# yhhshb/biolib

Hardware: AMD Instinct MI355X
Metric: Gbp/s minimizer-scanned (k=31,w=11) (higher is better)
Workload: dtype u64

## Files before the change

biolib_amd/csrc/bl_capi.hip:

```cpp
#include <hip/hip_runtime.h>
#include <algorithm>
#include <cstdio>
#include <cstdlib>
#include <cstring>
#include <deque>
#include <new>
#include <string>
#include <utility>
#include <vector>

#include "../../include/biolib_amd.h"
#include "bl_host.hpp"
#include "bl_launch.hpp"
#include "bl_lookup_launch.hpp"
#include "bl_read_counts_launch.hpp"
#include "bl_scan128_launch.hpp"

namespace {

thread_local std::string g_err;

int fail(int code, const std::string& msg)
{
    g_err = msg;
// ... 34 lines not shown
    size_t ws_bytes = 0;
    unsigned char* tile_buf = nullptr;
    size_t tile_buf_bytes = 0;
    uint16_t* slot_buf = nullptr;
    size_t slot_buf_bytes = 0;
    hipEvent_t ev_start = nullptr, ev_stop = nullptr;
    hipEvent_t ev_count_done = nullptr;
    bool count_recorded = false;
    bool scan_recorded = false;

    unsigned long long* shards() const { return reinterpret_cast<unsigned long long*>(ws + HDR_BYTES); }
    unsigned long long* result() const { return reinterpret_cast<unsigned long long*>(ws + HDR_BYTES + SHARD_BYTES); }
};

struct bl_ctx {
    int device = 0;
    Lane lanes[2];
    Lane* cur = nullptr;
    int next_lane = 0;
    int n_lanes = 1;
    uint32_t emit_lds_per_wg = 0;
    hipStream_t user_stream = nullptr;
    bool borrowed = false;
    hipStream_t stream = nullptr;
    unsigned long long* pinned = nullptr;
    hipEvent_t slot_ev[RING] = {};
    int next_slot = 0;
    std::deque<Pending> pending;
    bool timed = false;
    bool exact_windows = false;
    bool position_tiled = false;
    bool packed_codes = true;
    bool direct_codes = true;
    int jaccard128_path = 0;
    bool count128_tables = true;
    int table_prefix_bits = -1;
    bool ktiming = false;
    bl::LaunchLog last_kernels{};
    std::vector<hipEvent_t> ev_pool;
    std::vector<std::pair<hipEvent_t, hipEvent_t>> ev_open;
    double kernel_ms = 0.0;
    uint64_t kernel_launches = 0;
    std::vector<std::pair<hipEvent_t, hipEvent_t>> marks;
    std::vector<bl_batch*> batches;
    void* scratch[8] = {};
    size_t scratch_bytes[8] = {};
    std::vector<std::pair<void*, size_t>> pool_idle;
    std::vector<std::pair<void*, size_t>> pool_live;

    unsigned long long* shards() const { return cur->shards(); }
    unsigned long long* result() const { return cur->result(); }
    static size_t fixed_bytes() { return HDR_BYTES + SHARD_BYTES + RESULT_WORDS * sizeof(unsigned long long); }
};

struct bl_batch {
    bl_ctx* ctx = nullptr;
    uint8_t* bases = nullptr;
    bool owns_bases = false;
    uint32_t* start_bits = nullptr;
    uint32_t* packed = nullptr;
    uint32_t* codes = nullptr;
    uint32_t* chunk_bad = nullptr;
    uint64_t n_bases = 0;
    uint64_t n_seqs = 0;
    uint64_t read_len = 0;
    uint64_t origin = 0;
// ... 437 lines not shown

int bl_ctx_last_scan_ms(bl_ctx* c, float* ms)
{
    if (!c || !ms) return fail(BL_ERR_INVALID, "NULL argument");
    if (!c->timed) return fail(BL_ERR_INVALID, "no scan has been issued on this context");
    BL_HIP(hipEventSynchronize(c->cur->ev_stop));
    BL_HIP(hipEventElapsedTime(ms, c->cur->ev_start, c->cur->ev_stop));
    return BL_OK;
}

int bl_ctx_set_exact_windows(bl_ctx* c, int on)
{
    if (!c) return fail(BL_ERR_INVALID, "ctx is NULL");
    c->exact_windows = on != 0;
    return BL_OK;
}

int bl_ctx_set_option(bl_ctx* c, const char* name, int64_t value)
{
    if (!c || !name) return fail(BL_ERR_INVALID, "bl_ctx_set_option: NULL argument");
    const std::string n(name);
    if (n == "exact_windows" && (value == 0 || value == 1)) return bl_ctx_set_exact_windows(c, (int)value);
    if (n == "lanes") return bl_ctx_set_lanes(c, (int)value);
    if (n == "position_tiled" && (value == 0 || value == 1)) {
        c->position_tiled = value != 0;
        return BL_OK;
    }
    if (n == "packed_codes" && (value == 0 || value == 1)) {
        c->packed_codes = value != 0;
        return BL_OK;
    }
    if (n == "direct_codes" && (value == 0 || value == 1)) {
        c->direct_codes = value != 0;
        return BL_OK;
    }
    if (n == "count128_tables" && (value == 0 || value == 1)) {
        c->count128_tables = value != 0;
        return BL_OK;
    }
    if (n == "jaccard128_path" && value >= 0 && value <= 2) {
        c->jaccard128_path = (int)value;
        return BL_OK;
    }
    if (n == "table_prefix_bits" && value >= -1 && value <= bllk::MAX_PREFIX_BITS) {
        c->table_prefix_bits = (int)value;
        return BL_OK;
    }
    if (n == "emit_lds_bytes" && value >= 0 && value <= 160 * 1024) {
        c->emit_lds_per_wg = (uint32_t)value;
        return BL_OK;
    }
    return fail(BL_ERR_INVALID, "bl_ctx_set_option: unknown name or value out of range: " + n);
}

int bl_ctx_kernel_timing(bl_ctx* c, int enable)
{
    if (!c) return fail(BL_ERR_INVALID, "ctx is NULL");
    int rc = sync_ctx(c);
    if (rc != BL_OK) return rc;
    c->ktiming = enable != 0;
    c->kernel_ms = 0.0;
    c->kernel_launches = 0;
    return BL_OK;
}

int bl_ctx_kernel_time(bl_ctx* c, double* total_ms, uint64_t* launches)
// ... 527 lines not shown
{
    if (!c || !b || b->ctx != c) return fail(BL_ERR_INVALID, "ctx/batch is NULL or the batch belongs to another context");
    c->last_kernels.n = 0;
    if (unit < 1 || unit > bl::MAX_UNIT) return fail(BL_ERR_INVALID, "hashed unit length must be in [1, 32]");
    if (w < 1 || w > bl::MAX_W) return fail(BL_ERR_INVALID, "window must be in [1, 64]");
    uint64_t end;
    int rc = blh::range_end(b->n_bases, first, n, "a scan range", end);
    if (rc != BL_OK) return rc;
    if (end <= first) return zero_result(c, result, flags);
    p.bases = b->bases;
    p.n_bases = (int64_t)b->n_bases;
    p.pos_base = (int64_t)b->origin;
    p.exact_windows = c->exact_windows ? 1 : 0;
    bl::plan_scan(mode, (int64_t)first, (int64_t)end, (int)w, p);
    if (b->read_len && !c->position_tiled && !p.use_threshold && bl::frl_width_built(mode, (int)w)) {
        bl::plan_scan_frl_for(mode, (int64_t)first, (int64_t)end, (int64_t)b->n_bases, (int64_t)b->read_len, (int)unit, (int)w, (flags & BL_FLAG_CANONICAL) != 0, p);
    }
    if (!p.frl) {
        rc = ensure_start_bits(c, b);
        if (rc != BL_OK) return rc;
    }
    p.start_bits = b->start_bits;
    if (c->packed_codes && b->codes && bl::packed_covers(p) && (p.frl || bl::packed_scan_shape(mode, (int)w))) {
        p.codes_packed = b->codes;
        p.chunk_bad = b->chunk_bad;
        p.direct_codes = c->direct_codes ? 1 : 0;
    }
    p.unit = (int32_t)unit;
    p.w = (int32_t)w;
    p.seed = (uint32_t)seed;
    p.canonical = (flags & BL_FLAG_CANONICAL) ? 1 : 0;
    p.drop_last = (flags & BL_FLAG_DROP_LAST) ? 1 : 0;
    p.capacity = capacity;
    rc = begin_scan(c);
    if (rc != BL_OK) return rc;
    const size_t nt = (size_t)p.n_tiles, nb = (nt + bl::SCAN_BLK - 1) / bl::SCAN_BLK;
    rc = grow(c, reinterpret_cast<void**>(&c->cur->tile_buf), &c->cur->tile_buf_bytes, (2 * nt + 2 * nb + 8) * sizeof(unsigned long long) + nt * sizeof(uint32_t));
    if (rc != BL_OK) return rc;
    const size_t n_lists = mode == bl::MODE_SUPERKMER ? 3 : 1;
    const size_t slot_entries = nt * (size_t)p.stride;
    const size_t list_bytes = n_lists * slot_entries * sizeof(uint16_t);
    const size_t code_bytes = p.codes_packed ? 0 : nt * (size_t)p.slot_chunks * sizeof(uint32_t);
    rc = grow(c, reinterpret_cast<void**>(&c->cur->slot_buf), &c->cur->slot_buf_bytes, list_bytes + code_bytes);
    if (rc != BL_OK) return rc;
    unsigned long long* tb = reinterpret_cast<unsigned long long*>(c->cur->tile_buf);
    p.tile_counts = tb;
    p.tile_base = tb + nt;
    unsigned long long* block_tot = tb + 2 * nt;
    p.block_base = block_tot + nb;
    p.redo_list = reinterpret_cast<uint32_t*>(tb + 2 * nt + 2 * nb + 8);
    p.redo_count = reinterpret_cast<unsigned long long*>(c->cur->ws) + 1;
    p.slots_a = c->cur->slot_buf;
    p.slots_j = mode == bl::MODE_SUPERKMER ? c->cur->slot_buf + slot_entries : nullptr;
    p.slots_e = mode == bl::MODE_SUPERKMER ? c->cur->slot_buf + 2 * slot_entries : nullptr;
    p.slots_c = p.codes_packed ? nullptr : reinterpret_cast<uint32_t*>(reinterpret_cast<unsigned char*>(c->cur->slot_buf) + list_bytes);
    p.shards = c->shards();
    const bl::GroupRange all{0, (uint32_t)p.n_tiles};
    unsigned long long* carry = reinterpret_cast<unsigned long long*>(c->cur->ws);
    const bool staggered = c->n_lanes == 2 && !c->borrowed;
    if (staggered) {
        Lane* other = c->cur == &c->lanes[0] ? &c->lanes[1] : &c->lanes[0];
        if (other->count_recorded) BL_HIP(hipStreamWaitEvent(c->stream, other->ev_count_done, 0));
    }
    rc = kernel_event(c, true);
    if (rc != BL_OK) return rc;
    hipError_t e = bl::launch_scan_count(mode, p, all, c->stream, &c->last_kernels);
    if (e != hipSuccess) return fail(BL_ERR_HIP, std::string("scan_count_kernel: ") + hipGetErrorString(e));
    if (staggered) {
        BL_HIP(hipEventRecord(c->cur->ev_count_done, c->stream));
        c->cur->count_recorded = true;
    }
    rc = kernel_event(c, false);
    if (rc != BL_OK) return rc;
    e = bl::launch_tile_scan(p, all, block_tot, carry, c->stream);
    if (e != hipSuccess) return fail(BL_ERR_HIP, std::string("tile_scan: ") + hipGetErrorString(e));
    const uint32_t emit_lds_default = mode == bl::MODE_SUPERKMER ? 8192u : 28672u;
    e = bl::launch_scan_emit(mode, p, all, c->stream, staggered ? (c->emit_lds_per_wg ? c->emit_lds_per_wg : emit_lds_default) : 0, &c->last_kernels);
    if (e != hipSuccess) return fail(BL_ERR_HIP, std::string("scan_emit_kernel: ") + hipGetErrorString(e));
    return BL_OK;
}

int bl_scan_minimizers(bl_ctx* c, const bl_batch* b, uint64_t first, uint64_t n, uint32_t unit, uint32_t w, uint64_t seed, uint32_t flags,
                       uint64_t* d_values, uint64_t* d_positions, uint64_t* d_hashes, uint64_t capacity, bl_result* result)
{
    bl::ScanParams p{};
    p.out_value = d_values;
    p.out_pos = d_positions;
    p.out_hash = d_hashes;
    const bool wants = d_values || d_positions || d_hashes;
    int rc = scan_windows(bl::MODE_MINIMIZER, c, b, first, n, unit, w, seed, flags, p, wants ? capacity : 0, result);
    if (rc != BL_OK || p.n_tiles == 0) return rc;
    return end_scan(c, 1u << 0, result, wants, capacity, flags);
}

int bl_scan_hash_sample(bl_ctx* c, const bl_batch* b, uint64_t first, uint64_t n, uint32_t k, uint64_t seed, uint64_t threshold, uint32_t flags,
                        uint64_t* d_values, uint64_t* d_positions, uint64_t* d_hashes, uint64_t capacity, bl_result* result)
{
    bl::ScanParams p{};
    p.out_value = d_values;
    p.out_pos = d_positions;
    p.out_hash = d_hashes;
    p.use_threshold = 1;
// ... 164 lines not shown
```

biolib_amd/csrc/bl_kernels.hip:

```cpp
#include <hip/hip_runtime.h>
#include <cstdlib>
#include "bl_scan_frl.hpp"
#include "bl_launch.hpp"

#ifndef BL_SY0_WAVES
#define BL_SY0_WAVES 2
#endif
#ifndef BL_SY2_WAVES
#define BL_SY2_WAVES 3
#endif
#ifndef BL_CS_WAVES
#define BL_CS_WAVES 3
#endif
#ifndef BL_POSAX_WAVES
#define BL_POSAX_WAVES 4
#endif
#ifndef BL_SKAX_WAVES
#define BL_SKAX_WAVES 4
#endif
#ifndef BL_C4_WAVES
#define BL_C4_WAVES 5
#endif
#ifndef BL_CSRT_WAVES
#define BL_CSRT_WAVES 3
#endif

namespace bl {


__device__ __forceinline__ uint32_t wave_incl_scan_u32(uint32_t v, int lane)
{
    (void)lane;
#ifndef BL_SCAN_BUILTIN_DPP
// ... 170 lines not shown
        if (!PACKED) {
            uint32_t* sc = p.slots_c + (size_t)tile * p.slot_chunks;
            for (int c = tid; c < p.slot_chunks; c += TPB) sc[c] = sh.codes[c];
        }
        __syncthreads();
    }

    ThreadState st;
    bool tie = false;
    phase_hash_frl<MODE, W, NS, GENERIC, APPROX, U>(p, sh, tid, q0, tile, st, clean ? p.codes_packed + (q0 >> 4) : nullptr);
    phase_window_frl_a<MODE, W, NS, LIM_LAST, APPROX>(p, sh, tid, st, nullptr, &tie, clean);
    if (APPROX) {
        const bool any = wave_any(tie);
        if ((tid & 63) == 0) sh.wave_redo[wave_index(tid)] = any ? 1u : 0u;
    }
    const uint32_t packed = phase_window_frl_b<MODE, W, NS>(p, tid, st, nullptr);

    uint32_t total;
    const uint32_t excl = block_excl_scan(packed, sh.wave_tot, tid, total);
    const uint32_t n_s = total & 0xffffu, n_e = total >> 16;
    phase_list_frl<MODE, W, NS>(sh, st, excl & 0xffffu, excl >> 16);
    if (tid == 0) p.tile_counts[tile] = (unsigned long long)n_s | ((unsigned long long)n_e << 32);
    __syncthreads();
    if (APPROX && tid == 0 && BL_COLD((sh.wave_redo[0] | sh.wave_redo[1] | sh.wave_redo[2] | sh.wave_redo[3]) != 0)) p.redo_list[atomicAdd(p.redo_count, 1ull)] = tile;
    const size_t slot = (size_t)tile * p.stride;
    spill_list(p.slots_a + slot, sh.list_a, n_s, tid);
    if (MODE == MODE_SUPERKMER) {
        spill_list(p.slots_j + slot, sh.list_j, n_s, tid);
        spill_list(p.slots_e + slot, sh.list_e, n_e, tid);
    }
}

constexpr int C3_RC = NCHUNK + 4;
template <int MODE, bool LOOPED = false, bool C3 = false, bool WIDE = false, bool PACKED = false>
__device__ __forceinline__ void emit_tile(const ScanParams& p, uint32_t* codes, uint32_t tile, int tid, Digest& dg)
{
    const int64_t q0 = tile_q0(p, tile);
    const size_t slot = (size_t)tile * p.stride;
    const unsigned long long cnt = uniform64(p.tile_counts[tile]);
    const unsigned long long base = uniform64(p.tile_base[tile] + p.block_base[tile / SCAN_BLK]);
    const int needed = staged_chunks(p);
    const uint32_t* sc = PACKED ? p.codes_packed + (q0 >> 4) : p.slots_c + (size_t)tile * p.slot_chunks;
    const uint32_t c0 = (MODE != MODE_SYNCMER && tid < needed) ? sc[tid] : 0;
    const uint32_t c1 = (MODE != MODE_SYNCMER && TPB + tid < needed) ? sc[TPB + tid] : 0;
    const uint16_t* la = p.slots_a + slot;
    const uint16_t* lj = MODE == MODE_SUPERKMER ? p.slots_j + slot : nullptr;
    const bool in0 = tid < p.stride, in1 = TPB + tid < p.stride;
    const uint32_t a0 = in0 ? la[tid] : 0, a1 = in1 ? la[TPB + tid] : 0;
    uint32_t j0 = 0, j1 = 0;
    if (MODE == MODE_SUPERKMER) {
        j0 = in0 ? lj[tid] : 0;
        j1 = in1 ? lj[TPB + tid] : 0;
    }
    const uint32_t n_s = (uint32_t)cnt, n_e = (uint32_t)(cnt >> 32);
    if (n_s == 0 && n_e == 0) {
        if (LOOPED && MODE != MODE_SYNCMER) __syncthreads();
        return;
    }
    const uint64_t base_s = base & 0xffffffffull, base_e = base >> 32;
    if (C3) {
        if (tid < needed) {
            codes[1 + tid] = c0;
            codes[C3_RC + needed - tid] = revcomp16(c0);
        }
        if (TPB + tid < needed) {
            codes[1 + TPB + tid] = c1;
            codes[C3_RC + needed - TPB - tid] = revcomp16(c1);
        }
        __syncthreads();
    } else if (MODE != MODE_SYNCMER) {
        if (tid < needed) codes[tid] = c0;
        if (TPB + tid < needed) codes[TPB + tid] = c1;
        __syncthreads();
    }
    const bool fits = !BL_COLD(base_s + n_s > p.capacity);
    TileLists L{codes, la, lj, MODE == MODE_SUPERKMER ? p.slots_e + slot : nullptr, MODE == MODE_SUPERKMER ? p.slots_e + slot + p.stride : nullptr};
    const uint32_t d = (uint32_t)(base_s - base_e);
    auto one = [&](uint32_t r, uint32_t ent, uint32_t ent_j) {
        const Record rec = C3 ? emit_prepare_c3<LOOPED>(p, codes + 1, codes + C3_RC + 1, needed, q0, ent, dg) : emit_prepare<MODE, LOOPED>(p, codes, q0, ent, ent_j, dg);
        if (fits) emit_store<MODE, false>(p, rec, base_s + r);
        else emit_store<MODE, true>(p, rec, base_s + r);
        if (MODE == MODE_SUPERKMER && (p.out_size || p.out_records) && (fits || base_s + r < p.capacity)) {
            const int size = (int)(end_position(p, L, tile, q0, r + d, n_e) - (int64_t)rec.first + 1);
            if (p.out_size) p.out_size[base_s + r] = (uint8_t)size;
            if (WIDE) {
                if (p.out_records) emit_record128(p, codes, needed - 1, q0, rec, size, base_s + r);
            } else if (p.out_records) {
                emit_record(p, codes, needed - 1, q0, rec, size, base_s + r);
            }
        }
    };
    if ((uint32_t)tid < n_s) one(tid, a0, j0);
    if (LOOPED) BL_SCHED_FENCE();
    if ((uint32_t)(TPB + tid) < n_s) one(TPB + tid, a1, j1);
    if (LOOPED) BL_SCHED_FENCE();
#pragma unroll 1
    for (uint32_t r = 2 * TPB + tid; r < n_s; r += TPB) one(r, la[r], MODE == MODE_SUPERKMER ? lj[r] : 0u);
}

template <bool PACKED, int MODE, int W, int U, int C, int SY = 0>
__global__ __launch_bounds__(TPB, (MODE == MODE_MINIMIZER && SY == 2 ? BL_POSAX_WAVES : MODE == MODE_SUPERKMER && SY == 2 ? BL_SKAX_WAVES : SY == 1 && W < 0 ? BL_CSRT_WAVES : SY == 1 ? BL_CS_WAVES : SY == 2 ? BL_SY2_WAVES : (MODE == MODE_SYNCMER && W > 0 ? BL_SY0_WAVES : MODE == MODE_SYNCMER || (MODE == MODE_SUPERKMER && W == -32) ? 2 : (W == -32 || (W < 0 && MODE == MODE_SUPERKMER) ? 3 : (W == -16 ? 5 : (W < 0 ? 4 : (W <= 11 ? 5 : (MODE == MODE_SUPERKMER && W == 17 && U == 15 ? BL_C4_WAVES : 4)))))))) void scan_count_kernel(const ScanParams pin, GroupRange g)
{
    __shared__ TileShared<MODE, W> sh;
    ScanParams p = pin;
    if (U != 0) p.unit = U;
    if (W > 0) {
        p.w = W;
        p.stride = NWAVE * (64 * S - 16 * ((W + 15) / 16));
    }
// ... 45 lines not shown
#ifndef BL_FRL_WAVES
#define BL_FRL_WAVES 5
#endif
template <bool PACKED, int MODE, int W, int NS, int U, int L, int C, bool APPROX = false>
__global__ __launch_bounds__(TPB, (W <= 11 ? BL_FRL_WAVES : 4)) void scan_count_frl_kernel(const ScanParams pin, GroupRange g)
{
    __shared__ TileShared<MODE, W> sh;
    const ScanParams p = frl_params<MODE, W, NS, U, L, C>(pin);
    constexpr int LIM_LAST = frl_lim_last<W, NS, U, L>();
    static_assert(L == 0 || (LIM_LAST >= 1 && LIM_LAST <= NS), "read-tiled geometry: the last lane of a read must own 1..NS windows");
    if (blockIdx.x < g.count) count_tile_frl<MODE, W, NS, LIM_LAST, U == 0, APPROX, U, PACKED>(p, sh, g.first + blockIdx.x, threadIdx.x);
}

template <bool PACKED, int MODE, int W, int NS, int U, int L, int C>
__global__ __launch_bounds__(TPB, (W <= 11 ? 5 : 4)) void scan_redo_frl_kernel(const ScanParams pin)
{
    __shared__ TileShared<MODE, W> sh;
    const ScanParams p = frl_params<MODE, W, NS, U, L, C>(pin);
    const unsigned long long n = *p.redo_count;
    for (unsigned long long i = blockIdx.x; i < n; i += gridDim.x) {
        count_tile_frl<MODE, W, NS, frl_lim_last<W, NS, U, L>(), U == 0, false, U, PACKED>(p, sh, p.redo_list[i], threadIdx.x);
        __syncthreads();
    }
}

#ifndef BL_EMIT_TILES
#define BL_EMIT_TILES 4
#endif
template <int MODE>
constexpr int emit_tiles() { return MODE == MODE_MINIMIZER ? BL_EMIT_TILES : 1; }

template <int MODE, int U, int C, int FRL>
constexpr bool emit_c3() { return MODE == MODE_MINIMIZER && U == 31 && C == 1 && FRL == 1; }
template <int MODE, int U = 0, int C = -1, int FRL = -1, bool WIDE = false, bool PACKED = false>
__global__ __launch_bounds__(TPB) void scan_emit_kernel(const ScanParams pin, GroupRange g)
{
    static_assert(!WIDE || (MODE == MODE_SUPERKMER && U == 0), "32-byte records are super-k-mer groups; the unit length comes from the arguments");
    constexpr int K = emit_tiles<MODE>();
    constexpr bool C3 = emit_c3<MODE, U, C, FRL>();
    __shared__ uint32_t codes[K > 1 ? 2 : 1][C3 ? 2 * C3_RC : NCHUNK];
    const int tid = threadIdx.x;
    ScanParams p = pin;
    if (U != 0) p.unit = U;
    if (C >= 0) p.canonical = C;
    if (FRL >= 0) p.frl = FRL;
    Digest dg{0, 0, 0};
    if constexpr (K > 1) {
        __shared__ uint32_t acc[6][TPB];
#pragma unroll
        for (int i = 0; i < 6; ++i) acc[i][tid] = 0;
        const uint32_t t0 = blockIdx.x * K;
#pragma unroll 1
        for (uint32_t k = 0; k < (uint32_t)K && t0 + k < g.count; ++k) {
            Digest d1{0, 0, 0};
            emit_tile<MODE, true, C3, false, PACKED>(p, codes[k & 1], g.first + t0 + k, tid, d1);
            acc[0][tid] ^= (uint32_t)d1.xv; acc[1][tid] ^= (uint32_t)(d1.xv >> 32);
            acc[2][tid] ^= (uint32_t)d1.xh; acc[3][tid] ^= (uint32_t)(d1.xh >> 32);
            acc[4][tid] ^= (uint32_t)d1.xp; acc[5][tid] ^= (uint32_t)(d1.xp >> 32);
        }
        dg.xv = ((unsigned long long)acc[1][tid] << 32) | acc[0][tid];
        dg.xh = ((unsigned long long)acc[3][tid] << 32) | acc[2][tid];
        dg.xp = ((unsigned long long)acc[5][tid] << 32) | acc[4][tid];
    } else {
        if (blockIdx.x >= g.count) return;
        emit_tile<MODE, false, C3, WIDE, PACKED>(p, codes[0], g.first + blockIdx.x, tid, dg);
    }

    const unsigned long long xv = MODE == MODE_SYNCMER ? 0ull : wave_xor_to_last_u64(dg.xv), xh = MODE == MODE_SYNCMER ? 0ull : wave_xor_to_last_u64(dg.xh);
    const unsigned long long xp = wave_xor_to_last_u64(dg.xp);
    if ((tid & 63) == 63 && (xv | xh | xp)) {
        unsigned long long* shard = p.shards + 8 * ((blockIdx.x * NWAVE + (tid >> 6)) % NSHARD);
        if (MODE != MODE_SYNCMER) {
            atomicXor(&shard[1], xv);
            atomicXor(&shard[2], xh);
        }
        atomicXor(&shard[3], xp);
    }
}

__global__ __launch_bounds__(512) void tile_scan_local_kernel(const unsigned long long* counts, unsigned long long* tile_base,
                                                              unsigned long long* block_tot, uint32_t first_tile, uint32_t n_group)
{
    __shared__ unsigned long long wtot[8];
    const int tid = threadIdx.x, lane = tid & 63, wv = tid >> 6;
    const uint32_t rel = blockIdx.x * SCAN_BLK + tid * 4;
    unsigned long long c[4], run = 0;
#pragma unroll
    for (int i = 0; i < 4; ++i) {
// ... 188 lines not shown
    "frl<MM,W=11,NS=14,U=31,approx>", "frl_redo<MM,W=11,NS=14,U=31>", "frl<MM,W=11,NS=14,U=31>",
    "frl<MM,W=11,NS=15,U=31,approx>", "frl_redo<MM,W=11,NS=15,U=31>", "frl<MM,W=11,NS=15,U=31>",
    "frl<MM,W=11,NS=16,U=31,approx>", "frl_redo<MM,W=11,NS=16,U=31>", "frl<MM,W=11,NS=16,U=31>",
    "frl<MM,W=5>", "frl<MM,W=10>", "frl<MM,W=11>", "frl<MM,W=19>", "frl<SK,W=17>",
#ifndef BL_NO_POSAX
    "count<MM,W=11,U=31,C=1,approx>", "redo<MM,W=11,U=31,C=1>",
#endif
    "count<MM,W=11,U=31,C=1>",
#ifdef BL_SKAX
    "count<SK,W=17,U=15,C=1,approx>", "redo<SK,W=17,U=15,C=1>",
#endif
    "count<SK,W=17,U=15,C=1>",
    "count<SY,W=21,U=11,C=1,closed>", "redo<SY,W=21,U=11,C=1>",
#ifndef BL_NO_SY2
    "count<SY,W=21,U=11,C=1,deferred>",
#else
    "count<SY,W=21,U=11,C=1>",
#endif
    "count<SY,closed,W<=17>", "count<SY,closed,W<=32>",
#define BL_W(WV) "count<MM,W=" #WV ">", "count<SK,W=" #WV ">",
    BL_W_ALL(BL_W)
#undef BL_W
    "count<MM,W=1>", "count<SK,W=1>", "count<SY,W=1>", "count<SY,W=11>", "count<SY,W=17>", "count<SY,W=21>",
    "count<SY,W<=16>", "count<SY,W<=32>", "count<MM,W>32>", "count<SK,W>32>",
    "emit<MM>", "emit<SK>", "emit<SY>", "emit<MM,C3>", "emit<SK,wide>",
};

const char* const* scan_kernel_names(int* count)
{
    *count = (int)(sizeof(SCAN_KERNEL_NAMES) / sizeof(SCAN_KERNEL_NAMES[0]));
    return SCAN_KERNEL_NAMES;
}

static hipError_t launch_count_frl(int mode, const ScanParams& p, GroupRange g, hipStream_t stream, LaunchLog* log)
{
    const dim3 grid(g.count), block(TPB);
    if (mode == MODE_MINIMIZER && p.w == 11 && p.unit == 31 && p.canonical && p.read_len == 150 && p.ns == 15 && p.rpw == 8) {
        if (p.redo_list && g.first == 0 && !p.exact_windows) {
            BL_LAUNCH("frl<MM,W=11,NS=15,U=31,L=150,approx>", BL_PK(scan_count_frl_kernel, MODE_MINIMIZER, 11, 15, 31, 150, 1, true), grid, block, 0, p, g);
            BL_LAUNCH("frl_redo<MM,W=11,NS=15,U=31,L=150>", BL_PK(scan_redo_frl_kernel, MODE_MINIMIZER, 11, 15, 31, 150, 1), dim3(g.count < 512u ? g.count : 512u), block, 0, p);
        } else {
            BL_LAUNCH("frl<MM,W=11,NS=15,U=31,L=150>", BL_PK(scan_count_frl_kernel, MODE_MINIMIZER, 11, 15, 31, 150, 1), grid, block, 0, p, g);
        }
        return hipGetLastError();
    }
    if (mode == MODE_MINIMIZER && p.w == 11 && p.unit == 31 && p.canonical && p.ns >= 14 && p.ns <= 16) {
        const bool approx = p.redo_list && g.first == 0 && !p.exact_windows;
        const dim3 redo_grid(g.count < 512u ? g.count : 512u);
#define BL_FRL_SHAPE(NSV)                                                                                                                                    \
    if (approx) {                                                                                                                                            \
        BL_LAUNCH("frl<MM,W=11,NS=" #NSV ",U=31,approx>", BL_PK(scan_count_frl_kernel, MODE_MINIMIZER, 11, NSV, 31, 0, 1, true), grid, block, 0, p, g);            \
        BL_LAUNCH("frl_redo<MM,W=11,NS=" #NSV ",U=31>", BL_PK(scan_redo_frl_kernel, MODE_MINIMIZER, 11, NSV, 31, 0, 1), redo_grid, block, 0, p);                   \
    } else {                                                                                                                                                 \
        BL_LAUNCH("frl<MM,W=11,NS=" #NSV ",U=31>", BL_PK(scan_count_frl_kernel, MODE_MINIMIZER, 11, NSV, 31, 0, 1), grid, block, 0, p, g);                         \
    }
        if (p.ns == 14) { BL_FRL_SHAPE(14) } else if (p.ns == 15) { BL_FRL_SHAPE(15) } else { BL_FRL_SHAPE(16) }
#undef BL_FRL_SHAPE
        return hipGetLastError();
    }
    if (p.ns != S) return hipErrorInvalidValue;
    if (mode == MODE_MINIMIZER) {
        switch (p.w) {
            case 5: BL_LAUNCH("frl<MM,W=5>", BL_PK(scan_count_frl_kernel, MODE_MINIMIZER, 5, S, 0, 0, -1), grid, block, 0, p, g); break;
            case 10: BL_LAUNCH("frl<MM,W=10>", BL_PK(scan_count_frl_kernel, MODE_MINIMIZER, 10, S, 0, 0, -1), grid, block, 0, p, g); break;
            case 11: BL_LAUNCH("frl<MM,W=11>", BL_PK(scan_count_frl_kernel, MODE_MINIMIZER, 11, S, 0, 0, -1), grid, block, 0, p, g); break;
            case 19: BL_LAUNCH("frl<MM,W=19>", BL_PK(scan_count_frl_kernel, MODE_MINIMIZER, 19, S, 0, 0, -1), grid, block, 0, p, g); break;
            default: return hipErrorInvalidValue;
        }
    } else if (mode == MODE_SUPERKMER && p.w == 17) {
        BL_LAUNCH("frl<SK,W=17>", BL_PK(scan_count_frl_kernel, MODE_SUPERKMER, 17, S, 0, 0, -1), grid, block, 0, p, g);
    } else {
        return hipErrorInvalidValue;
    }
    return hipGetLastError();
}

template <int MODE>
static hipError_t launch_count_mode(const ScanParams& p, GroupRange g, hipStream_t stream, LaunchLog* log)
{
    const dim3 grid(g.count), block(TPB);
    if (MODE == MODE_MINIMIZER && p.w == 11 && p.unit == 31 && p.canonical) {
#ifndef BL_NO_POSAX
        if (p.redo_list && g.first == 0 && !p.exact_windows) {
            BL_LAUNCH("count<MM,W=11,U=31,C=1,approx>", BL_PK(scan_count_kernel, MODE_MINIMIZER, 11, 31, 1, 2), grid, block, 0, p, g);
            BL_LAUNCH("redo<MM,W=11,U=31,C=1>", BL_PK(scan_redo_kernel, MODE_MINIMIZER, 11, 31, 1), dim3(g.count < 512u ? g.count : 512u), block, 0, p);
            return hipGetLastError();
        }
#endif
        BL_LAUNCH("count<MM,W=11,U=31,C=1>", BL_PK(scan_count_kernel, MODE, 11, 31, 1), grid, block, 0, p, g);
        return hipGetLastError();
    }
// ... 23 lines not shown
            BL_LAUNCH("count<SY,W=21,U=11,C=1>", BL_PK(scan_count_kernel, MODE, 21, 11, 1), grid, block, 0, p, g);
        }
        return hipGetLastError();
    }
    if (MODE == MODE_SYNCMER && p.w <= 32 && !p.exact_windows && ((p.soff == 0 && p.eoff == p.w - 1) || (p.soff == p.w - 1 && p.eoff == 0))) {
        if (p.w <= 17) BL_LAUNCH("count<SY,closed,W<=17>", BL_PK(scan_count_kernel, MODE_SYNCMER, -8, 0, -1, 1), grid, block, 0, p, g);
        else BL_LAUNCH("count<SY,closed,W<=32>", BL_PK(scan_count_kernel, MODE_SYNCMER, -16, 0, -1, 1), grid, block, 0, p, g);
        return hipGetLastError();
    }
    if (MODE != MODE_SYNCMER && p.w >= 2 && p.w <= 32) {
        constexpr int MM = MODE == MODE_SYNCMER ? MODE_MINIMIZER : MODE;
        switch (p.w) {
#define BL_W(WV) case WV: BL_LAUNCH(BL_MODE_NAME("count<", ",W=" #WV ">"), BL_PK_W(scan_count_kernel, MM, WV, 0, -1), grid, block, 0, p, g); return hipGetLastError();
            BL_W_ALL(BL_W)
#undef BL_W
        }
    }
    switch (p.w) {
        case 1: BL_LAUNCH(BL_MODE_NAME("count<", ",W=1>"), BL_PK(scan_count_kernel, MODE, 1, 0, -1), grid, block, 0, p, g); break;
        case 11: BL_LAUNCH(BL_MODE_NAME("count<", ",W=11>"), BL_PK(scan_count_kernel, MODE, 11, 0, -1), grid, block, 0, p, g); break;
        case 17: BL_LAUNCH(BL_MODE_NAME("count<", ",W=17>"), BL_PK(scan_count_kernel, MODE, 17, 0, -1), grid, block, 0, p, g); break;
        case 21: BL_LAUNCH(BL_MODE_NAME("count<", ",W=21>"), BL_PK(scan_count_kernel, MODE, 21, 0, -1), grid, block, 0, p, g); break;
        default:
            if constexpr (MODE == MODE_SYNCMER) {
                if (p.w <= 16) { BL_LAUNCH("count<SY,W<=16>", BL_PK(scan_count_kernel, MODE, -8, 0, -1), grid, block, 0, p, g); break; }
                if (p.w <= 32) { BL_LAUNCH("count<SY,W<=32>", BL_PK(scan_count_kernel, MODE, -16, 0, -1), grid, block, 0, p, g); break; }
            }
            BL_LAUNCH(BL_MODE_NAME("count<", ",W>32>"), BL_PK(scan_count_kernel, MODE, -32, 0, -1), grid, block, 0, p, g);
            break;
    }
    return hipGetLastError();
}

hipError_t launch_scan_count(int mode, const ScanParams& p, GroupRange g, hipStream_t stream, LaunchLog* log)
{
    if (g.count == 0) return hipSuccess;
    if (p.frl) return launch_count_frl(mode, p, g, stream, log);
    switch (mode) {
        case MODE_MINIMIZER: return launch_count_mode<MODE_MINIMIZER>(p, g, stream, log);
        case MODE_SUPERKMER: return launch_count_mode<MODE_SUPERKMER>(p, g, stream, log);
        case MODE_SYNCMER: return launch_count_mode<MODE_SYNCMER>(p, g, stream, log);
    }
    return hipErrorInvalidValue;
}

template <int MODE>
static void launch_emit_mode(const ScanParams& p, GroupRange g, hipStream_t stream, uint32_t lds_per_wg, LaunchLog* log)
{
    constexpr int K = emit_tiles<MODE>();
    const uint32_t have = (uint32_t)(((K > 1 ? 2 : 1) * NCHUNK + (K > 1 ? 6 * TPB : 0)) * sizeof(uint32_t));
    const uint32_t pad = lds_per_wg > have ? lds_per_wg - have : 0;
    const dim3 grid((g.count + K - 1) / K), block(TPB);
    if (MODE == MODE_MINIMIZER && p.frl && p.unit == 31 && p.canonical) {
        const uint32_t have_c3 = (uint32_t)(((K > 1 ? 2 : 1) * 2 * C3_RC + (K > 1 ? 6 * TPB : 0)) * sizeof(uint32_t));
        if (p.codes_packed) BL_LAUNCH("emit<MM,C3>", (scan_emit_kernel<MODE_MINIMIZER, 31, 1, 1, false, true>), grid, block, lds_per_wg > have_c3 ? lds_per_wg - have_c3 : 0, p, g);
        else BL_LAUNCH("emit<MM,C3>", (scan_emit_kernel<MODE_MINIMIZER, 31, 1, 1>), grid, block, lds_per_wg > have_c3 ? lds_per_wg - have_c3 : 0, p, g);
        return;
    }
    if (MODE == MODE_SUPERKMER && p.records128) {
        if (p.codes_packed) BL_LAUNCH("emit<SK,wide>", (scan_emit_kernel<MODE_SUPERKMER, 0, -1, -1, true, true>), grid, block, pad, p, g);
        else BL_LAUNCH("emit<SK,wide>", (scan_emit_kernel<MODE_SUPERKMER, 0, -1, -1, true>), grid, block, pad, p, g);
        return;
    }
    if (MODE != MODE_SYNCMER && p.codes_packed) BL_LAUNCH(BL_MODE_NAME("emit<", ">"), (scan_emit_kernel<MODE, 0, -1, -1, false, MODE != MODE_SYNCMER>), grid, block, pad, p, g);
    else BL_LAUNCH(BL_MODE_NAME("emit<", ">"), (scan_emit_kernel<MODE>), grid, block, pad, p, g);
}

hipError_t launch_scan_emit(int mode, const ScanParams& p, GroupRange g, hipStream_t stream, uint32_t lds_per_wg, LaunchLog* log)
{
    if (g.count == 0) return hipSuccess;
    switch (mode) {
        case MODE_MINIMIZER: launch_emit_mode<MODE_MINIMIZER>(p, g, stream, lds_per_wg, log); break;
        case MODE_SUPERKMER: launch_emit_mode<MODE_SUPERKMER>(p, g, stream, lds_per_wg, log); break;
        case MODE_SYNCMER: launch_emit_mode<MODE_SYNCMER>(p, g, stream, lds_per_wg, log); break;
        default: return hipErrorInvalidValue;
    }
    return hipGetLastError();
}
#undef BL_LAUNCH
#undef BL_PK
#undef BL_PK_W
#undef BL_MODE_NAME
#undef BL_W_ALL

hipError_t launch_tile_scan(const ScanParams& p, GroupRange g, unsigned long long* block_tot, unsigned long long* carry, hipStream_t stream)
{
    if (g.count == 0) return hipSuccess;
    const uint32_t n_blocks = (g.count + SCAN_BLK - 1) / SCAN_BLK;
    hipLaunchKernelGGL(tile_scan_local_kernel, dim3(n_blocks), dim3(512), 0, stream, p.tile_counts, p.tile_base, block_tot, g.first, g.count);
// ... 59 lines not shown
```

biolib_amd/csrc/bl_launch.hpp:

```cpp
#pragma once
#include <hip/hip_runtime.h>
#include "bl_scan_phases.hpp"

namespace bl {
struct LaunchLog {
    static constexpr int MAX = 8;
    const char* names[MAX];
    int n;
    void add(const char* name) { if (n < MAX) names[n++] = name; }
};
const char* const* scan_kernel_names(int* count);
hipError_t launch_scan_count(int mode, const ScanParams& p, GroupRange g, hipStream_t stream, LaunchLog* log);
hipError_t launch_scan_emit(int mode, const ScanParams& p, GroupRange g, hipStream_t stream, uint32_t lds_per_wg, LaunchLog* log);
hipError_t launch_tile_scan(const ScanParams& p, GroupRange g, unsigned long long* block_tot, unsigned long long* carry, hipStream_t stream);
hipError_t launch_kmers(const KmerParams& p, int n_blocks, hipStream_t stream);
hipError_t launch_reduce_shards(const unsigned long long* shards, unsigned long long* result, uint32_t add_mask, const unsigned long long* redone, hipStream_t stream);
hipError_t launch_synth(uint8_t* bases, uint64_t first, uint64_t n, uint64_t seed, hipStream_t stream);
hipError_t launch_start_bits_fixed(uint32_t* bits, uint64_t n_words, uint64_t n_bases, uint64_t read_len, hipStream_t stream);
hipError_t launch_start_bits_offsets(uint32_t* bits, const uint64_t* offsets, uint64_t n_seqs, uint64_t n_bases, hipStream_t stream);
hipError_t launch_pack_codes(const uint8_t* bases, uint64_t n_bases, uint32_t* codes, uint32_t* chunk_bad, hipStream_t stream);
}
```

biolib_amd/csrc/bl_scan_core.hpp:

```cpp
#pragma once
#include <stdint.h>

#if defined(__HIPCC__) && !defined(BL_CPU_EMU)
#define BL_DEV __host__ __device__ __forceinline__
#define BL_UNROLL _Pragma("unroll")
#else
#define BL_DEV static inline
#define BL_UNROLL
#endif

#ifdef BL_CENSUS_HOT
#define BL_COLD(c) (false)
#else
#define BL_COLD(c) (c)
#endif

#if defined(__HIP_DEVICE_COMPILE__) && !defined(BL_CPU_EMU) && !defined(BL_NO_SCHED_FENCE)
#define BL_SCHED_FENCE() __builtin_amdgcn_sched_barrier(0)
#else
#define BL_SCHED_FENCE() do {} while (0)
#endif

namespace bl {

// ... 26 lines not shown
    int32_t drop_last;
    int32_t use_threshold;
    uint64_t hash_below;
    uint64_t* out_value;
    uint64_t* out_pos;
    uint64_t* out_hash;
    uint64_t* out_first;
    uint8_t* out_mmpos;
    uint8_t* out_size;
    uint64_t* out_records;
    uint64_t capacity;
    unsigned long long* tile_counts;
    unsigned long long* tile_base;
    unsigned long long* block_base;
    uint16_t* slots_a;
    uint16_t* slots_j;
    uint16_t* slots_e;
    uint32_t* slots_c;
    int32_t slot_chunks;
    unsigned long long* shards;
    int32_t exact_windows;
    uint32_t* redo_list;
    unsigned long long* redo_count;
    int32_t frl;
    int32_t read_len;
    int32_t lpr, rpw, ns;
    int32_t nwin;
    uint32_t lpr_inv;
    int64_t n_reads;
    int32_t records128;
    const uint32_t* codes_packed;
    const uint32_t* chunk_bad;
    int32_t direct_codes;
};

constexpr int PACK_LEAD = 32, PACK_TAIL = NCHUNK;
BL_DEV int64_t packed_total(int64_t n_bases) { return (PACK_LEAD + ((n_bases + 15) >> 4) + PACK_TAIL + 63) & ~63LL; }
constexpr bool packed_scan_shape(int mode, int w) { return !(mode == MODE_MINIMIZER && w == 25); }
BL_DEV bool packed_covers(const ScanParams& p)
{
    return p.n_tiles > 0 && p.origin >= -16 * (int64_t)PACK_LEAD && p.origin + (int64_t)(p.n_tiles - 1) * p.stride < p.n_bases + 16;
}

BL_DEV bool frl_width_built(int mode, int w)
{
    return (mode == MODE_MINIMIZER && (w == 11 || w == 5 || w == 10 || w == 19)) || (mode == MODE_SUPERKMER && w == 17);
}

BL_DEV bool plan_scan_frl(int64_t first, int64_t end, int64_t n_bases, int64_t read_len, int unit, int w, int ns_fixed, ScanParams& p)
{
    if (read_len <= 0 || read_len > 4096 || first % read_len != 0) return false;
    if (end % read_len != 0 || end > n_bases || end <= first) return false;
    const int L = (int)read_len;
    const int nu = L - unit + 1, nwin = nu - w + 1;
    if (nwin < 1 || w < 2) return false;
    const int lpr = (nu + S - 1) / S;
    if (lpr > 64) return false;
    const int ns = ns_fixed ? ns_fixed : (nu + lpr - 1) / lpr;
    if (ns * lpr < nu || ns > S || w - 1 > 3 * ns) return false;
    int rpw = 64 / lpr;
    const int cap = (NCHUNK * 16 - 64 - 32) / NWAVE_CORE / L;
    if (rpw > cap) rpw = cap;
    if (rpw < 1) return false;
    const double frl_eff = (double)(rpw * nwin) / (64.0 * ns);
    const double pos_eff = (double)nwin / L * (double)(64 * S - 16 * ((w + 15) / 16)) / (64.0 * S);
    if (frl_eff <= pos_eff) return false;
// ... 583 lines not shown
```

biolib_amd/csrc/bl_scan_phases.hpp:

```cpp
#pragma once
#include <type_traits>

#include "bl_scan_core.hpp"

namespace bl {

constexpr int NWAVE = TPB / 64;
constexpr int WH = 64 * S;
constexpr int WCHUNK = 64 + 8;

template <int MODE, int W>
struct TileShared {
    uint32_t codes[NCHUNK];
    uint32_t flags[NCHUNK];
    typename std::conditional<(MODE == MODE_SYNCMER || W == -32), uint64_t, uint32_t>::type half[W < 0 ? S : 1][W < 0 ? TPB : 1];
    alignas(4) uint16_t list_a[H];
    alignas(4) uint16_t list_j[MODE == MODE_SUPERKMER ? H : 2];
    alignas(4) uint16_t list_e[MODE == MODE_SUPERKMER ? H : 2];
    uint32_t wave_tot[NWAVE];
    uint32_t redo;
    uint32_t wave_bad[NWAVE];
    uint32_t wave_redo[NWAVE];
    unsigned long long dig[4];
};
// ... 1064 lines not shown
    Record rec{0, 0, 0, 0, 0};
    const int wv = p.frl ? 0 : ent >> 12, ap = p.frl ? ent : ent & 0xfff;
    const int64_t wq0 = p.frl ? q0 : wave_origin(p, q0, wv);
    rec.pos = (uint64_t)(wq0 + ap);
    dg.xp ^= rec.pos + (uint64_t)p.pos_base;
    if (MODE != MODE_SYNCMER) {
        rec.v = extract_unit(p.frl ? codes : codes + wave_chunk0(p, wv), ap, p.unit, p.canonical);
        if (FENCED) BL_SCHED_FENCE();
        rec.h = murmur64(rec.v, p.seed);
        if (FENCED) BL_SCHED_FENCE();
        dg.xv ^= rec.v;
        dg.xh ^= rec.h;
        if (MODE == MODE_SUPERKMER) {
            const int j = p.frl ? ent_j : ent_j & 0xfff;
            rec.first = (uint64_t)(wq0 + j);
            rec.mmpos = (uint32_t)(ap - j);
        }
    }
    return rec;
}

template <bool FENCED = false>
BL_DEV uint64_t unit31_canonical(const uint32_t* cf, const uint32_t* cr, int nc, int pos)
{
    const int qf = (pos + 30) >> 4, qr = nc - 1 - (pos >> 4);
    const int shf = 2 - 2 * pos, shr = 2 * pos;
    const uint32_t flo = funnel_shr(cf[qf - 1], cf[qf], shf & 31), fhi = funnel_shr(cf[qf - 2], cf[qf - 1], shf & 31) & 0x3fffffffu;
    if (FENCED) BL_SCHED_FENCE();
    const uint32_t rlo = funnel_shr(cr[qr - 1], cr[qr], shr & 31), rhi = funnel_shr(cr[qr - 2], cr[qr - 1], shr & 31) & 0x3fffffffu;
    const uint64_t fw = ((uint64_t)fhi << 32) | flo, rv = ((uint64_t)rhi << 32) | rlo;
    return min62<31>(rv, fw);
}

template <bool FENCED = false>
BL_DEV Record emit_prepare_c3(const ScanParams& p, const uint32_t* cf, const uint32_t* cr, int nc, int64_t q0, uint32_t ent, Digest& dg)
{
    Record rec{0, 0, 0, 0, 0};
    rec.pos = (uint64_t)(q0 + (int)ent);
    dg.xp ^= rec.pos + (uint64_t)p.pos_base;
    rec.v = unit31_canonical<FENCED>(cf, cr, nc, (int)ent);
    if (FENCED) BL_SCHED_FENCE();
    rec.h = murmur64(rec.v, p.seed);
    if (FENCED) BL_SCHED_FENCE();
    dg.xv ^= rec.v;
    dg.xh ^= rec.h;
    return rec;
}

template <typename T>
BL_DEV void stream_store(T* dst, T v)
{
#if defined(__HIP_DEVICE_COMPILE__) && !defined(BL_CPU_EMU)
    __builtin_nontemporal_store(v, dst);
#else
    *dst = v;
#endif
}

template <int MODE, bool CHECK = true>
BL_DEV void emit_store(const ScanParams& p, const Record& rec, uint64_t g)
{
    if (CHECK && g >= p.capacity) return;
    if (MODE == MODE_SYNCMER) {
        if (p.out_pos) stream_store(&p.out_pos[g], rec.pos + (uint64_t)p.pos_base);
        return;
    }
    if (p.out_value) stream_store(&p.out_value[g], rec.v);
    if (p.out_hash) stream_store(&p.out_hash[g], rec.h);
    if (p.out_pos) stream_store(&p.out_pos[g], rec.pos + (uint64_t)p.pos_base);
    if (MODE == MODE_SUPERKMER) {
        if (p.out_first) stream_store(&p.out_first[g], rec.first + (uint64_t)p.pos_base);
        if (p.out_mmpos) p.out_mmpos[g] = (uint8_t)rec.mmpos;
    }
}

BL_DEV void emit_record(const ScanParams& p, const uint32_t* codes, int last_chunk, int64_t q0, const Record& rec, int size, uint64_t g)
{
    uint64_t x, y;
    pack_group(codes, last_chunk, (int)((int64_t)rec.first - q0), size + p.unit + p.w - 2, rec.mmpos, size, x, y);
    stream_store(&p.out_records[2 * g], x);
    stream_store(&p.out_records[2 * g + 1], y);
}

BL_DEV void emit_record128(const ScanParams& p, const uint32_t* codes, int last_chunk, int64_t q0, const Record& rec, int size, uint64_t g)
{
    uint64_t w[4];
    pack_group128(codes, last_chunk, (int)((int64_t)rec.first - q0), size + p.unit + p.w - 2, rec.mmpos, size, w);
#if defined(__HIP_DEVICE_COMPILE__) && !defined(BL_CPU_EMU)
    typedef uint64_t u64x2 __attribute__((ext_vector_type(2)));
    u64x2* dst = reinterpret_cast<u64x2*>(p.out_records + 4 * g);
    u64x2 lo, hi;
    lo.x = w[0]; lo.y = w[1];
    hi.x = w[2]; hi.y = w[3];
    __builtin_nontemporal_store(lo, dst);
    __builtin_nontemporal_store(hi, dst + 1);
#else
    for (int i = 0; i < 4; ++i) p.out_records[4 * g + i] = w[i];
#endif
}

template <int MODE>
BL_DEV void phase_emit(const ScanParams& p, const TileLists& L, uint32_t tile, int tid, int64_t q0, uint32_t n_s, uint32_t n_e, uint64_t base_s, uint64_t base_e,
                       Digest& dg)
{
    const bool fits = !BL_COLD(base_s + n_s > p.capacity);
    const uint32_t d = (uint32_t)(base_s - base_e);
// ... 82 lines not shown
```

Measured before the change: 616.0.

## Use uniform-base lane-offset stores in C3 emit and record count event earlier

Adds a scalar-store path to the C3 minimizer emit kernel. Each round computes uniform output base pointers once and stores through a per-lane 32-bit byte offset, with the opaque-VGPR asm keeping the offset in a vector register so the compiler can use scalar-base addressing. Positions are computed with 32-bit arithmetic plus a rare carry fix, and an unchecked all-outputs store path is used when the tile fits capacity. Separately, the count-done event is now recorded right after the approximate count kernel, before the redo kernel, so the other lane can start earlier. The change adds code complexity and depends on compiler codegen behaving as intended.

```diff
diff --git a/biolib_amd/csrc/bl_capi.hip b/biolib_amd/csrc/bl_capi.hip
--- a/biolib_amd/csrc/bl_capi.hip
+++ b/biolib_amd/csrc/bl_capi.hip
@@ -90,6 +90,8 @@
     bool position_tiled = false;
     bool packed_codes = true;
     bool direct_codes = true;
+    bool scalar_stores = true;
+    bool early_count_event = true;
     int jaccard128_path = 0;
     bool count128_tables = true;
     int table_prefix_bits = -1;
@@ -593,6 +595,14 @@
     }
     if (n == "direct_codes" && (value == 0 || value == 1)) {
         c->direct_codes = value != 0;
+        return BL_OK;
+    }
+    if (n == "scalar_stores" && (value == 0 || value == 1)) {
+        c->scalar_stores = value != 0;
+        return BL_OK;
+    }
+    if (n == "early_count_event" && (value == 0 || value == 1)) {
+        c->early_count_event = value != 0;
         return BL_OK;
     }
     if (n == "count128_tables" && (value == 0 || value == 1)) {
@@ -1186,6 +1196,7 @@
     p.canonical = (flags & BL_FLAG_CANONICAL) ? 1 : 0;
     p.drop_last = (flags & BL_FLAG_DROP_LAST) ? 1 : 0;
     p.capacity = capacity;
+    p.scalar_stores = c->scalar_stores ? 1 : 0;
     rc = begin_scan(c);
     if (rc != BL_OK) return rc;
     const size_t nt = (size_t)p.n_tiles, nb = (nt + bl::SCAN_BLK - 1) / bl::SCAN_BLK;
@@ -1218,10 +1229,11 @@
     }
     rc = kernel_event(c, true);
     if (rc != BL_OK) return rc;
-    hipError_t e = bl::launch_scan_count(mode, p, all, c->stream, &c->last_kernels);
+    const bool early = staggered && c->early_count_event;
+    hipError_t e = bl::launch_scan_count(mode, p, all, c->stream, &c->last_kernels, early ? c->cur->ev_count_done : nullptr);
     if (e != hipSuccess) return fail(BL_ERR_HIP, std::string("scan_count_kernel: ") + hipGetErrorString(e));
     if (staggered) {
-        BL_HIP(hipEventRecord(c->cur->ev_count_done, c->stream));
+        if (!early) BL_HIP(hipEventRecord(c->cur->ev_count_done, c->stream));
         c->cur->count_recorded = true;
     }
     rc = kernel_event(c, false);
diff --git a/biolib_amd/csrc/bl_kernels.hip b/biolib_amd/csrc/bl_kernels.hip
--- a/biolib_amd/csrc/bl_kernels.hip
+++ b/biolib_amd/csrc/bl_kernels.hip
@@ -1,4 +1,5 @@
 #include <hip/hip_runtime.h>
+#include <type_traits>
 #include <cstdlib>
 #include "bl_scan_frl.hpp"
 #include "bl_launch.hpp"
@@ -235,7 +236,7 @@
 }
 
 constexpr int C3_RC = NCHUNK + 4;
-template <int MODE, bool LOOPED = false, bool C3 = false, bool WIDE = false, bool PACKED = false>
+template <int MODE, bool LOOPED = false, bool C3 = false, bool WIDE = false, bool PACKED = false, bool SS = false>
 __device__ __forceinline__ void emit_tile(const ScanParams& p, uint32_t* codes, uint32_t tile, int tid, Digest& dg)
 {
     const int64_t q0 = tile_q0(p, tile);
@@ -278,6 +279,28 @@
     }
     const bool fits = !BL_COLD(base_s + n_s > p.capacity);
     TileLists L{codes, la, lj, MODE == MODE_SUPERKMER ? p.slots_e + slot : nullptr, MODE == MODE_SUPERKMER ? p.slots_e + slot + p.stride : nullptr};
+    if constexpr (C3 && SS) {
+        const int64_t q0_out = q0 + p.pos_base;
+        const uint32_t lane_off = 8u * (uint32_t)tid;
+        auto rounds = [&](auto ALL) {
+            auto round = [&](uint32_t r0, uint32_t ent) {
+                const Record rec = emit_prepare_c3<LOOPED, true>(p, codes + 1, codes + C3_RC + 1, needed, q0_out, ent, dg);
+                const EmitBases b = emit_bases(p, base_s + r0);
+                if (decltype(ALL)::value) emit_store_lane_all(b, rec, lane_off);
+                else emit_store_lane(b, rec, tid, lane_off, emit_room(p, base_s + r0));
+            };
+            if ((uint32_t)tid < n_s) round(0, a0);
+            if (LOOPED) BL_SCHED_FENCE();
+            if ((uint32_t)(TPB + tid) < n_s) round(TPB, a1);
+            if (LOOPED) BL_SCHED_FENCE();
+#pragma unroll 1
+            for (uint32_t r0 = 2 * TPB; r0 < n_s; r0 += TPB)
+                if (r0 + (uint32_t)tid < n_s) round(r0, la[r0 + tid]);
+        };
+        if (fits && p.out_value && p.out_hash && p.out_pos) rounds(std::true_type{});
+        else rounds(std::false_type{});
+        return;
+    }
     const uint32_t d = (uint32_t)(base_s - base_e);
     auto one = [&](uint32_t r, uint32_t ent, uint32_t ent_j) {
         const Record rec = C3 ? emit_prepare_c3<LOOPED>(p, codes + 1, codes + C3_RC + 1, needed, q0, ent, dg) : emit_prepare<MODE, LOOPED>(p, codes, q0, ent, ent_j, dg);
@@ -389,12 +412,13 @@
 
 template <int MODE, int U, int C, int FRL>
 constexpr bool emit_c3() { return MODE == MODE_MINIMIZER && U == 31 && C == 1 && FRL == 1; }
-template <int MODE, int U = 0, int C = -1, int FRL = -1, bool WIDE = false, bool PACKED = false>
+template <int MODE, int U = 0, int C = -1, int FRL = -1, bool WIDE = false, bool PACKED = false, bool SS = false>
 __global__ __launch_bounds__(TPB) void scan_emit_kernel(const ScanParams pin, GroupRange g)
 {
     static_assert(!WIDE || (MODE == MODE_SUPERKMER && U == 0), "32-byte records are super-k-mer groups; the unit length comes from the arguments");
     constexpr int K = emit_tiles<MODE>();
     constexpr bool C3 = emit_c3<MODE, U, C, FRL>();
+    static_assert(!SS || C3, "the scalar store form is built for the C3 record kernel");
     __shared__ uint32_t codes[K > 1 ? 2 : 1][C3 ? 2 * C3_RC : NCHUNK];
     const int tid = threadIdx.x;
     ScanParams p = pin;
@@ -410,7 +434,7 @@
 #pragma unroll 1
         for (uint32_t k = 0; k < (uint32_t)K && t0 + k < g.count; ++k) {
             Digest d1{0, 0, 0};
-            emit_tile<MODE, true, C3, false, PACKED>(p, codes[k & 1], g.first + t0 + k, tid, d1);
+            emit_tile<MODE, true, C3, false, PACKED, SS>(p, codes[k & 1], g.first + t0 + k, tid, d1);
             acc[0][tid] ^= (uint32_t)d1.xv; acc[1][tid] ^= (uint32_t)(d1.xv >> 32);
             acc[2][tid] ^= (uint32_t)d1.xh; acc[3][tid] ^= (uint32_t)(d1.xh >> 32);
             acc[4][tid] ^= (uint32_t)d1.xp; acc[5][tid] ^= (uint32_t)(d1.xp >> 32);
@@ -665,17 +689,26 @@
     return SCAN_KERNEL_NAMES;
 }
 
-static hipError_t launch_count_frl(int mode, const ScanParams& p, GroupRange g, hipStream_t stream, LaunchLog* log)
-{
+static hipError_t launch_count_frl(int mode, const ScanParams& p, GroupRange g, hipStream_t stream, LaunchLog* log, hipEvent_t& count_done)
+{
+    hipError_t ev_err = hipSuccess;
+#define BL_COUNT_DONE()                                        \
+    do {                                                       \
+        if (count_done) {                                      \
+            ev_err = hipEventRecord(count_done, stream);       \
+            count_done = nullptr;                              \
+        }                                                      \
+    } while (0)
     const dim3 grid(g.count), block(TPB);
     if (mode == MODE_MINIMIZER && p.w == 11 && p.unit == 31 && p.canonical && p.read_len == 150 && p.ns == 15 && p.rpw == 8) {
         if (p.redo_list && g.first == 0 && !p.exact_windows) {
             BL_LAUNCH("frl<MM,W=11,NS=15,U=31,L=150,approx>", BL_PK(scan_count_frl_kernel, MODE_MINIMIZER, 11, 15, 31, 150, 1, true), grid, block, 0, p, g);
+            BL_COUNT_DONE();
             BL_LAUNCH("frl_redo<MM,W=11,NS=15,U=31,L=150>", BL_PK(scan_redo_frl_kernel, MODE_MINIMIZER, 11, 15, 31, 150, 1), dim3(g.count < 512u ? g.count : 512u), block, 0, p);
         } else {
             BL_LAUNCH("frl<MM,W=11,NS=15,U=31,L=150>", BL_PK(scan_count_frl_kernel, MODE_MINIMIZER, 11, 15, 31, 150, 1), grid, block, 0, p, g);
         }
-        return hipGetLastError();
+        return ev_err != hipSuccess ? ev_err : hipGetLastError();
     }
     if (mode == MODE_MINIMIZER && p.w == 11 && p.unit == 31 && p.canonical && p.ns >= 14 && p.ns <= 16) {
         const bool approx = p.redo_list && g.first == 0 && !p.exact_windows;
@@ -683,13 +716,15 @@
 #define BL_FRL_SHAPE(NSV)                                                                                                                                    \
     if (approx) {                                                                                                                                            \
         BL_LAUNCH("frl<MM,W=11,NS=" #NSV ",U=31,approx>", BL_PK(scan_count_frl_kernel, MODE_MINIMIZER, 11, NSV, 31, 0, 1, true), grid, block, 0, p, g);            \
+        BL_COUNT_DONE();                                                                                                                                     \
         BL_LAUNCH("frl_redo<MM,W=11,NS=" #NSV ",U=31>", BL_PK(scan_redo_frl_kernel, MODE_MINIMIZER, 11, NSV, 31, 0, 1), redo_grid, block, 0, p);                   \
     } else {                                                                                                                                                 \
         BL_LAUNCH("frl<MM,W=11,NS=" #NSV ",U=31>", BL_PK(scan_count_frl_kernel, MODE_MINIMIZER, 11, NSV, 31, 0, 1), grid, block, 0, p, g);                         \
     }
         if (p.ns == 14) { BL_FRL_SHAPE(14) } else if (p.ns == 15) { BL_FRL_SHAPE(15) } else { BL_FRL_SHAPE(16) }
 #undef BL_FRL_SHAPE
-        return hipGetLastError();
+#undef BL_COUNT_DONE
+        return ev_err != hipSuccess ? ev_err : hipGetLastError();
     }
     if (p.ns != S) return hipErrorInvalidValue;
     if (mode == MODE_MINIMIZER) {
@@ -779,16 +814,21 @@
     return hipGetLastError();
 }
 
-hipError_t launch_scan_count(int mode, const ScanParams& p, GroupRange g, hipStream_t stream, LaunchLog* log)
-{
-    if (g.count == 0) return hipSuccess;
-    if (p.frl) return launch_count_frl(mode, p, g, stream, log);
-    switch (mode) {
-        case MODE_MINIMIZER: return launch_count_mode<MODE_MINIMIZER>(p, g, stream, log);
-        case MODE_SUPERKMER: return launch_count_mode<MODE_SUPERKMER>(p, g, stream, log);
-        case MODE_SYNCMER: return launch_count_mode<MODE_SYNCMER>(p, g, stream, log);
-    }
-    return hipErrorInvalidValue;
+hipError_t launch_scan_count(int mode, const ScanParams& p, GroupRange g, hipStream_t stream, LaunchLog* log, hipEvent_t count_done)
+{
+    if (g.count == 0) return count_done ? hipEventRecord(count_done, stream) : hipSuccess;
+    hipError_t e = hipErrorInvalidValue;
+    if (p.frl) {
+        e = launch_count_frl(mode, p, g, stream, log, count_done);
+    } else {
+        switch (mode) {
+            case MODE_MINIMIZER: e = launch_count_mode<MODE_MINIMIZER>(p, g, stream, log); break;
+            case MODE_SUPERKMER: e = launch_count_mode<MODE_SUPERKMER>(p, g, stream, log); break;
+            case MODE_SYNCMER: e = launch_count_mode<MODE_SYNCMER>(p, g, stream, log); break;
+        }
+    }
+    if (e == hipSuccess && count_done) e = hipEventRecord(count_done, stream);
+    return e;
 }
 
 template <int MODE>
@@ -800,8 +840,11 @@
     const dim3 grid((g.count + K - 1) / K), block(TPB);
     if (MODE == MODE_MINIMIZER && p.frl && p.unit == 31 && p.canonical) {
         const uint32_t have_c3 = (uint32_t)(((K > 1 ? 2 : 1) * 2 * C3_RC + (K > 1 ? 6 * TPB : 0)) * sizeof(uint32_t));
-        if (p.codes_packed) BL_LAUNCH("emit<MM,C3>", (scan_emit_kernel<MODE_MINIMIZER, 31, 1, 1, false, true>), grid, block, lds_per_wg > have_c3 ? lds_per_wg - have_c3 : 0, p, g);
-        else BL_LAUNCH("emit<MM,C3>", (scan_emit_kernel<MODE_MINIMIZER, 31, 1, 1>), grid, block, lds_per_wg > have_c3 ? lds_per_wg - have_c3 : 0, p, g);
+        const uint32_t pad_c3 = lds_per_wg > have_c3 ? lds_per_wg - have_c3 : 0;
+        if (p.codes_packed && p.scalar_stores) BL_LAUNCH("emit<MM,C3>", (scan_emit_kernel<MODE_MINIMIZER, 31, 1, 1, false, true, true>), grid, block, pad_c3, p, g);
+        else if (p.codes_packed) BL_LAUNCH("emit<MM,C3>", (scan_emit_kernel<MODE_MINIMIZER, 31, 1, 1, false, true>), grid, block, pad_c3, p, g);
+        else if (p.scalar_stores) BL_LAUNCH("emit<MM,C3>", (scan_emit_kernel<MODE_MINIMIZER, 31, 1, 1, false, false, true>), grid, block, pad_c3, p, g);
+        else BL_LAUNCH("emit<MM,C3>", (scan_emit_kernel<MODE_MINIMIZER, 31, 1, 1>), grid, block, pad_c3, p, g);
         return;
     }
     if (MODE == MODE_SUPERKMER && p.records128) {
diff --git a/biolib_amd/csrc/bl_launch.hpp b/biolib_amd/csrc/bl_launch.hpp
--- a/biolib_amd/csrc/bl_launch.hpp
+++ b/biolib_amd/csrc/bl_launch.hpp
@@ -10,7 +10,7 @@
     void add(const char* name) { if (n < MAX) names[n++] = name; }
 };
 const char* const* scan_kernel_names(int* count);
-hipError_t launch_scan_count(int mode, const ScanParams& p, GroupRange g, hipStream_t stream, LaunchLog* log);
+hipError_t launch_scan_count(int mode, const ScanParams& p, GroupRange g, hipStream_t stream, LaunchLog* log, hipEvent_t count_done = nullptr);
 hipError_t launch_scan_emit(int mode, const ScanParams& p, GroupRange g, hipStream_t stream, uint32_t lds_per_wg, LaunchLog* log);
 hipError_t launch_tile_scan(const ScanParams& p, GroupRange g, unsigned long long* block_tot, unsigned long long* carry, hipStream_t stream);
 hipError_t launch_kmers(const KmerParams& p, int n_blocks, hipStream_t stream);
diff --git a/biolib_amd/csrc/bl_scan_core.hpp b/biolib_amd/csrc/bl_scan_core.hpp
--- a/biolib_amd/csrc/bl_scan_core.hpp
+++ b/biolib_amd/csrc/bl_scan_core.hpp
@@ -82,6 +82,7 @@
     const uint32_t* codes_packed;
     const uint32_t* chunk_bad;
     int32_t direct_codes;
+    int32_t scalar_stores;
 };
 
 constexpr int PACK_LEAD = 32, PACK_TAIL = NCHUNK;
diff --git a/biolib_amd/csrc/bl_scan_phases.hpp b/biolib_amd/csrc/bl_scan_phases.hpp
--- a/biolib_amd/csrc/bl_scan_phases.hpp
+++ b/biolib_amd/csrc/bl_scan_phases.hpp
@@ -1120,12 +1120,22 @@
     return min62<31>(rv, fw);
 }
 
-template <bool FENCED = false>
+template <bool FENCED = false, bool POS32 = false>
 BL_DEV Record emit_prepare_c3(const ScanParams& p, const uint32_t* cf, const uint32_t* cr, int nc, int64_t q0, uint32_t ent, Digest& dg)
 {
     Record rec{0, 0, 0, 0, 0};
-    rec.pos = (uint64_t)(q0 + (int)ent);
-    dg.xp ^= rec.pos + (uint64_t)p.pos_base;
+    if (POS32) {
+        const uint32_t qlo = (uint32_t)q0, lo = qlo + ent;
+        rec.pos = ((uint64_t)q0 & 0xffffffff00000000ull) | lo;
+        if (BL_COLD(qlo > 0xffff0000u)) {
+            BL_SCHED_FENCE();
+            rec.pos += (uint64_t)(lo < qlo ? 1u : 0u) << 32;
+        }
+        dg.xp ^= rec.pos;
+    } else {
+        rec.pos = (uint64_t)(q0 + (int)ent);
+        dg.xp ^= rec.pos + (uint64_t)p.pos_base;
+    }
     rec.v = unit31_canonical<FENCED>(cf, cr, nc, (int)ent);
     if (FENCED) BL_SCHED_FENCE();
     rec.h = murmur64(rec.v, p.seed);
@@ -1160,6 +1170,51 @@
         if (p.out_first) stream_store(&p.out_first[g], rec.first + (uint64_t)p.pos_base);
         if (p.out_mmpos) p.out_mmpos[g] = (uint8_t)rec.mmpos;
     }
+}
+
+struct EmitBases {
+    uint64_t *v, *h, *pos;
+};
+BL_DEV EmitBases emit_bases(const ScanParams& p, uint64_t g)
+{
+    return EmitBases{p.out_value ? p.out_value + g : nullptr, p.out_hash ? p.out_hash + g : nullptr, p.out_pos ? p.out_pos + g : nullptr};
+}
+BL_DEV int32_t emit_room(const ScanParams& p, uint64_t g)
+{
+    return g >= p.capacity ? 0 : (p.capacity - g > 0x7fffffffull ? 0x7fffffff : (int32_t)(p.capacity - g));
+}
+#if defined(__HIP_DEVICE_COMPILE__) && !defined(BL_CPU_EMU)
+#define BL_OPAQUE_VGPR(x) asm volatile("" : "+v"(x))
+#else
+#define BL_OPAQUE_VGPR(x) do {} while (0)
+#endif
+template <typename T>
+BL_DEV void stream_store_lane(T* base, uint32_t lane_off, T v)
+{
+    stream_store(reinterpret_cast<T*>(reinterpret_cast<unsigned char*>(base) + lane_off), v);
+}
+BL_DEV void emit_store_lane(const EmitBases& b, const Record& rec, int tid, uint32_t lane_off, int32_t room)
+{
+    if (tid >= room) return;
+    if (b.v) {
+        BL_OPAQUE_VGPR(lane_off);
+        stream_store_lane(b.v, lane_off, rec.v);
+    }
+    if (b.h) {
+        BL_OPAQUE_VGPR(lane_off);
+        stream_store_lane(b.h, lane_off, rec.h);
+    }
+    if (b.pos) {
+        BL_OPAQUE_VGPR(lane_off);
+        stream_store_lane(b.pos, lane_off, rec.pos);
+    }
+}
+BL_DEV void emit_store_lane_all(const EmitBases& b, const Record& rec, uint32_t lane_off)
+{
+    BL_OPAQUE_VGPR(lane_off);
+    stream_store_lane(b.v, lane_off, rec.v);
+    stream_store_lane(b.h, lane_off, rec.h);
+    stream_store_lane(b.pos, lane_off, rec.pos);
 }
 
 BL_DEV void emit_record(const ScanParams& p, const uint32_t* codes, int last_chunk, int64_t q0, const Record& rec, int size, uint64_t g)
```

After: 621.0 (median of 6 runs). About the same (+0.8%).
